# annegnx/PnP-Flow

Hardware: AMD Instinct MI355X
Metric: restored images/sec (higher is better)
Workload: dtype f32-equivalent (f16 hi+lo split operands, 3 x f16 MFMA per product, f32 accumulate); 1 GPU; CelebA-shaped 256x256 box-inpainting (half-size 40, sigma 0.05) pnp_flow B=32/GPU 100x5 (the configuration BASELINE.json's metric is quoted on; main.py:132-136 at 256^2); image=256x256x3, batch_per_gpu=32, global_batch=32, steps_pnp=100, num_samples=5, weights=synthetic seed 0 (no checkpoint offline), hipgraph=True, unet_batch=160, parallelism=dp1 (contiguous shards of the global batch, no data-path collective)

## Files before the change

pnpflow_amd/csrc/conv_pp.hip:

```cpp
#include "pp_common.h"

namespace pf {

constexpr int pp_a9(int MT) { return (pp_npix(MT) * 8 + 255) / 256; }

#ifdef PP_PROBE_BUILD
__device__ unsigned long long* g_pp_dbg = nullptr;
__device__ int g_pp_dbg_skip = 0;
#define PP_STAMP(k) do { if (stamp_buf != nullptr && blockIdx.x == 0 && t == 0 && stamp_n >= 0 && stamp_n < 64) stamp_buf[(team * 64 + stamp_n) * 8 + (k)] = __builtin_readcyclecounter(); } while (0)
#else
#define PP_STAMP(k) do { } while (0)
#endif

template <int MT, int N9, int N1, bool RES, int TEAMS = 2, int TERMS = 3>
__global__ __launch_bounds__(256 * TEAMS, 2) void conv_pp_kernel(const PPParams p) {
    constexpr int NCH = N9 + N1;
    constexpr int W9 = pp_w9(TERMS), W1 = pp_w1(TERMS), WSTEP = TERMS == 3 ? 2048 : 1024;
    static_assert(TERMS == 3 || TERMS == 1, "split terms");
    constexpr int PP_NPIX = pp_npix(MT), PP_PATCH_BYTES = pp_patch_bytes(MT), PP_A9 = pp_a9(MT), TH = 8 * MT;
    constexpr int LASTN = PP_NPIX * 8 - (PP_A9 - 1) * 256;
    constexpr int WBYTES = N9 * W9 + N1 * W1;
    static_assert(NCH >= 1 && NCH <= PP_MAXCH && N9 >= 1, "chunk structure");
    extern __shared__ __attribute__((aligned(16))) char smem[];
    const int tid = threadIdx.x;
    const int team = TEAMS == 2 ? __builtin_amdgcn_readfirstlane(tid >> 8) : 0;
    const int t = tid & 255, lane = t & 63, wm = __builtin_amdgcn_readfirstlane(t >> 6);
    const int l31 = lane & 31, hi = lane >> 5;
    const unsigned patch0 = (unsigned)WBYTES + (unsigned)team * PP_PATCH_BYTES;
    const pp_float_cptr scale_c = (pp_float_cptr)(uintptr_t)p.scale;
    auto wlds = [](int c) constexpr { return c < N9 ? c * W9 : N9 * W9 + (c - N9) * W1; };

#pragma unroll
    for (int c = 0; c < NCH; ++c) {
        const uint4* src = reinterpret_cast<const uint4*>(p.ch[c].wimg);
        uint4* dst = reinterpret_cast<uint4*>(smem + wlds(c));
        const int n16 = (c < N9 ? 9 : 1) * 256;
        if constexpr (TERMS == 3) {
            for (int i = tid; i < n16; i += 256 * TEAMS) dst[i] = src[i];
        } else {
            for (int i = tid; i < n16 / 2; i += 256 * TEAMS) dst[i] = src[(i >> 6) * 128 + (i & 63)];
        }
    }

    const int qi = t & 7, p0 = t >> 3;
    unsigned pk9[PP_A9];
#pragma unroll
    for (int i = 0; i < PP_A9; ++i) {
        const int pp = min(p0 + 32 * i, PP_NPIX - 1);
        const int py = pp / PP_PW, px = pp - py * PP_PW;
// ... 26 lines not shown

    const int G = gridDim.x;
    const int rg = (blockIdx.x & 7) * (G >> 3) + (blockIdx.x >> 3);
    const int T = p.B << (p.lx + p.ly);
    const int t_begin = (int)((long)rg * T / G), t_end = (int)((long)(rg + 1) * T / G);
    const int ntl = t_end - t_begin;
    const int niter = (ntl + TEAMS - 1) / TEAMS;
    const int rot = ntl > 0 ? (int)(((long)rg * p.rot) % ntl) : 0;
    auto tile_of = [&](int it) __attribute__((always_inline)) -> PPTile {
        const int idx = min(it * TEAMS + team, ntl - 1);
        const int wrapped = idx + rot >= ntl ? idx + rot - ntl : idx + rot;
        const int tl = t_begin + wrapped;
        PPTile r;
        const int tx = tl & ((1 << p.lx) - 1), ty = (tl >> p.lx) & ((1 << p.ly) - 1);
        r.b = tl >> (p.lx + p.ly); r.oy0 = ty * TH; r.ox0 = tx * 16;
        r.edge = (ty == 0 ? 1 : 0) | (ty == (1 << p.ly) - 1 ? 2 : 0) | (tx == 0 ? 4 : 0) | (tx == (1 << p.lx) - 1 ? 8 : 0);
        return r;
    };
    auto live_of = [&](int it) __attribute__((always_inline)) -> bool { return it >= 0 && (t_begin + it * TEAMS + team) < t_end; };

    struct Pre {
        float4 ra[PP_A9];
        float4 csc, csh;
        float ascale;
        unsigned inval;
    };
    Pre pre0, pre1;
    struct Res { float4 rv[MT][4]; float addv; };
    static_assert(MT == 1, "conv_pp_kernel: the residual / accumulator scheme below is the one of 8 x 16-pixel team tiles");
    constexpr int RD = 2;
    constexpr int NRES = NCH == 1 ? 2 : 1;
    Res res0, res1;

    auto issue_patch = [&](Pre& S, const PPTile& tl, auto C_) __attribute__((always_inline)) {
        constexpr int C = decltype(C_)::value;
        const long bpix = ((long)tl.b * p.H + tl.oy0) * p.W + tl.ox0;
        const int cstride = p.ch[C].cstride;
        S.ascale = p.scale != nullptr ? scale_c[8 * tl.b + p.ch[C].seg] : 1.0f;
        const unsigned cs4 = (unsigned)cstride * 4u, q16 = (unsigned)qi * 16u;
        if constexpr (C < N9) {
            const char* base = reinterpret_cast<const char*>(p.ch[C].src + (bpix - p.W - 1) * cstride + p.ch[C].coff);
            unsigned inval = 0;
#pragma unroll
            for (int i = 0; i < PP_A9; ++i) inval |= (((pk9[i] >> 20) & (unsigned)tl.edge) != 0u ? 1u : 0u) << i;
            S.inval = inval;
            const char* cb = reinterpret_cast<const char*>(p.coef + (size_t)tl.b * 2 * p.coef_stride + p.ch[C].gn_c0);
            S.csc = *reinterpret_cast<const float4*>(cb + q16); S.csh = *reinterpret_cast<const float4*>(cb + (unsigned)(p.coef_stride * 4) + q16);
#pragma unroll
            for (int i = 0; i < PP_A9; ++i) {
                const unsigned px = ((inval >> i) & 1u) ? (unsigned)pix_safe : (pk9[i] & 0xffffu);
                S.ra[i] = *reinterpret_cast<const float4*>(base + (__umul24(px, cs4) + q16));
            }
        } else {
            const char* base = reinterpret_cast<const char*>(p.ch[C].src + bpix * cstride + p.ch[C].coff);
            S.inval = 0;
#pragma unroll
            for (int i = 0; i < TH / 2; ++i) S.ra[i] = *reinterpret_cast<const float4*>(base + (__umul24((unsigned)(pixoff1 + 2 * i * p.W), cs4) + q16));
        }
    };

    auto split_store = [&](float4 v, unsigned addr) __attribute__((always_inline)) {
        if constexpr (TERMS == 3) {
            uint2 h, l;
            split4_pp(v, h.x, h.y, l.x, l.y);
            *reinterpret_cast<uint2*>(smem + addr) = h;
            *reinterpret_cast<uint2*>(smem + (addr ^ 64u)) = l;
        } else {
            uint2 h;
            asm("v_cvt_pk_f16_f32 %0, %2, %3\n\tv_cvt_pk_f16_f32 %1, %4, %5" : "=&v"(h.x), "=&v"(h.y) : "v"(v.x), "v"(v.y), "v"(v.z), "v"(v.w));
            *reinterpret_cast<uint2*>(smem + addr) = h;
        }
    };

    auto stage_and_request = [&](Pre& S, auto C_, const PPTile& t2, auto C2_) __attribute__((always_inline)) {
        constexpr int C = decltype(C_)::value, C2 = decltype(C2_)::value;
        constexpr int NT_ = C < N9 ? PP_A9 : TH / 2, NL_ = C2 < N9 ? PP_A9 : TH / 2;
        const long bpix = ((long)t2.b * p.H + t2.oy0) * p.W + t2.ox0;
        const int cstride = p.ch[C2].cstride;
        const unsigned cs4 = (unsigned)cstride * 4u, q16 = (unsigned)qi * 16u;
        const char* base = reinterpret_cast<const char*>(p.ch[C2].src + (bpix - (C2 < N9 ? p.W + 1 : 0)) * cstride + p.ch[C2].coff);
        unsigned inval2 = 0;
        if constexpr (C2 < N9) {
#pragma unroll
            for (int i = 0; i < PP_A9; ++i) inval2 |= (((pk9[i] >> 20) & (unsigned)t2.edge) != 0u ? 1u : 0u) << i;
        }
        const bool silu = C < N9 ? p.ch[C].xform == 2 : false;
#pragma unroll
        for (int i = 0; i < (NT_ > NL_ ? NT_ : NL_); ++i) {
            if (i < NT_) {
                float4 v = S.ra[i];
                if constexpr (C < N9) {
                    v.x = v.x * S.csc.x + S.csh.x; v.y = v.y * S.csc.y + S.csh.y; v.z = v.z * S.csc.z + S.csh.z; v.w = v.w * S.csc.w + S.csh.w;
                    if (silu) silu4_pp(v);
                    const float f = ((S.inval >> i) & 1u) ? 0.0f : S.ascale;
                    v.x *= f; v.y *= f; v.z *= f; v.w *= f;
                    if (i < PP_A9 - 1 || t < LASTN) split_store(v, ldsw9 + (unsigned)(i * 4096) + (((pk9[i] >> 16) & 7u) << 4));
                } else {
                    v.x *= S.ascale; v.y *= S.ascale; v.z *= S.ascale; v.w *= S.ascale;
                    split_store(v, ldsw1 + (unsigned)(2 * i * PP_PW * 128));
                }
            }
            if (i < NL_) {
                if constexpr (C2 < N9) {
                    const unsigned px = ((inval2 >> i) & 1u) ? (unsigned)pix_safe : (pk9[i] & 0xffffu);
                    S.ra[i] = *reinterpret_cast<const float4*>(base + (__umul24(px, cs4) + q16));
                } else {
                    S.ra[i] = *reinterpret_cast<const float4*>(base + (__umul24((unsigned)(pixoff1 + 2 * i * p.W), cs4) + q16));
                }
            }
        }
        S.inval = inval2;
        S.ascale = p.scale != nullptr ? scale_c[8 * t2.b + p.ch[C2].seg] : 1.0f;
        if constexpr (C2 < N9) {
            const char* cb = reinterpret_cast<const char*>(p.coef + (size_t)t2.b * 2 * p.coef_stride + p.ch[C2].gn_c0);
            S.csc = *reinterpret_cast<const float4*>(cb + q16); S.csh = *reinterpret_cast<const float4*>(cb + (unsigned)(p.coef_stride * 4) + q16);
        }
    };

    constexpr int NACC = 2;
    f32x16 acc[NACC][MT];
#pragma unroll
    for (int mt = 0; mt < MT; ++mt)
#pragma unroll
        for (int r = 0; r < 16; ++r) { for (int a = 0; a < NACC; ++a) acc[a][mt][r] = 0.f; }
    float run1[4] = {0.f, 0.f, 0.f, 0.f}, run2[4] = {0.f, 0.f, 0.f, 0.f};
    int run_b = -1, run_n = 0;

    auto mma_step = [&](unsigned wbase, int s, int ky, int kx, int j) __attribute__((always_inline)) {
        const int ai = (s & 1) % NACC;
        if constexpr (TERMS == 3) {
            const f16x8 bh = *reinterpret_cast<const f16x8*>(smem + wbase + (unsigned)((s * 2 + 0) * 1024));
            const f16x8 bl = *reinterpret_cast<const f16x8*>(smem + wbase + (unsigned)((s * 2 + 1) * 1024));
            f16x8 ah[MT], al[MT];
#pragma unroll
            for (int mt = 0; mt < MT; ++mt) {
                const unsigned off = (unsigned)((mt * 2 + ky) * PP_PW * 128);
                ah[mt] = *reinterpret_cast<const f16x8*>(smem + a_addr[kx][j][0] + off);
                al[mt] = *reinterpret_cast<const f16x8*>(smem + a_addr[kx][j][1] + off);
            }
#pragma unroll
            for (int mt = 0; mt < MT; ++mt) acc[ai][mt] = __builtin_amdgcn_mfma_f32_32x32x16_f16(al[mt], bh, acc[ai][mt], 0, 0, 0);
#pragma unroll
            for (int mt = 0; mt < MT; ++mt) acc[ai][mt] = __builtin_amdgcn_mfma_f32_32x32x16_f16(ah[mt], bl, acc[ai][mt], 0, 0, 0);
#pragma unroll
            for (int mt = 0; mt < MT; ++mt) acc[ai][mt] = __builtin_amdgcn_mfma_f32_32x32x16_f16(ah[mt], bh, acc[ai][mt], 0, 0, 0);
        } else {
            const f16x8 bh = *reinterpret_cast<const f16x8*>(smem + wbase + (unsigned)(s * WSTEP));
#pragma unroll
            for (int mt = 0; mt < MT; ++mt) {
                const f16x8 ah = *reinterpret_cast<const f16x8*>(smem + a_addr[kx][j][0] + (unsigned)((mt * 2 + ky) * PP_PW * 128));
                acc[ai][mt] = __builtin_amdgcn_mfma_f32_32x32x16_f16(ah, bh, acc[ai][mt], 0, 0, 0);
            }
        }
    };

    auto flush_stats = [&]() __attribute__((always_inline)) {
        if (p.stats_out == nullptr || run_b < 0) return;
#pragma unroll
        for (int j = 0; j < 4; ++j) {
            double a = (double)run1[j], q = (double)run2[j];
            a += __shfl_xor(a, 8); q += __shfl_xor(q, 8);
            a += __shfl_xor(a, 16); q += __shfl_xor(q, 16);
            a += __shfl_xor(a, 32); q += __shfl_xor(q, 32);
            if (lane < 8) {
                double* dst = p.stats_out + ((size_t)run_b * 32 + em * 4 + j) * 2;
                unsafeAtomicAdd(dst, a); unsafeAtomicAdd(dst + 1, q);
            }
            run1[j] = 0.f; run2[j] = 0.f;
        }
        run_n = 0;
    };

    auto epilogue = [&](const Res& R, const PPTile& tl, bool live) __attribute__((always_inline)) {
        if (!live) return;
        if (tl.b != run_b || run_n >= 32) { flush_stats(); run_b = tl.b; }
        ++run_n;
        const float inv_last = p.scale != nullptr ? scale_c[8 * tl.b + 4 + p.ch[NCH - 1].seg] : 1.0f;
        const float oscale = p.out_scale * (1.0f / 256.0f) * inv_last;
        float* obase = p.out + (((size_t)tl.b * p.H + tl.oy0 + wm * 2 * MT) * p.W + tl.ox0) * 32;
#pragma unroll
        for (int mt = 0; mt < MT; ++mt) {
            float e[16];
#pragma unroll
            for (int r = 0; r < 16; ++r) e[r] = (NACC == 2 ? acc[0][mt][r] + acc[NACC - 1][mt][r] : acc[0][mt][r]) * oscale + R.addv;
#pragma unroll
            for (int g = 0; g < 4; ++g) {
                oct_transpose(e[4 * g], e[4 * g + 1], e[4 * g + 2], e[4 * g + 3], bit3);
                float4 v = make_float4(e[4 * g], e[4 * g + 1], e[4 * g + 2], e[4 * g + 3]);
                if constexpr (RES) {
                    const float rsc = p.res_scale; const float4 r4 = R.rv[mt][g];
                    v.x = fmaf(r4.x, rsc, v.x); v.y = fmaf(r4.y, rsc, v.y); v.z = fmaf(r4.z, rsc, v.z); v.w = fmaf(r4.w, rsc, v.w);
                }
                char* dst = reinterpret_cast<char*>(obase) + (size_t)((mt * 2 + (g >> 1)) * p.W) * 128 + (g & 1) * 1024 + e_lane;
                nt_store4(dst, v);
                run1[0] += v.x; run1[1] += v.y; run1[2] += v.z; run1[3] += v.w;
                run2[0] += v.x * v.x; run2[1] += v.y * v.y; run2[2] += v.z * v.z; run2[3] += v.w * v.w;
            }
        }
    };

    auto issue_res = [&](Res& R, const PPTile& tl) __attribute__((always_inline)) {
        R.addv = p.addvec != nullptr ? p.addvec[(size_t)tl.b * p.addvec_bs + ch_of_col] : 0.f;
        if constexpr (RES) {
            const char* rbase = reinterpret_cast<const char*>(p.residual + (((size_t)tl.b * p.H + tl.oy0 + wm * 2 * MT) * p.W + tl.ox0) * 32);
#pragma unroll
            for (int mt = 0; mt < MT; ++mt)
#pragma unroll
                for (int g = 0; g < 4; ++g)
                    R.rv[mt][g] = nt_load4(rbase + (size_t)((mt * 2 + (g >> 1)) * p.W) * 128 + (g & 1) * 1024 + e_lane);
        }
    };

    auto mma_chunk = [&](const PPTile& tl, auto C_) __attribute__((always_inline)) {
        constexpr int C = decltype(C_)::value;
        if constexpr (C == 0) {
#pragma unroll
            for (int mt = 0; mt < MT; ++mt)
#pragma unroll
                for (int r = 0; r < 16; ++r) { for (int a = 0; a < NACC; ++a) acc[a][mt][r] = 0.f; }
        } else {
            if (p.scale != nullptr && p.ch[C - 1].seg != p.ch[C].seg) {
                const float ratio = scale_c[8 * tl.b + p.ch[C].seg] * scale_c[8 * tl.b + 4 + p.ch[C - 1].seg];
                if (ratio != 1.0f) {
#pragma unroll
                    for (int mt = 0; mt < MT; ++mt)
#pragma unroll
                        for (int r = 0; r < 16; ++r) { for (int a = 0; a < NACC; ++a) acc[a][mt][r] *= ratio; }
                }
            }
        }
        const unsigned wbase = (unsigned)wlds(C) + b_lane;
        __builtin_amdgcn_s_setprio(1);
        if constexpr (C < N9) {
#pragma unroll
            for (int tap = 0; tap < 9; ++tap)
#pragma unroll
                for (int j = 0; j < 2; ++j) mma_step(wbase, tap * 2 + j, tap / 3, tap % 3, j);
        } else {
#pragma unroll
            for (int j = 0; j < 2; ++j) mma_step(wbase, j, 1, 1, j);
        }
        __builtin_amdgcn_s_setprio(0);
    };

    int stamp_n = 0; (void)stamp_n;
#ifdef PP_PROBE_BUILD
    unsigned long long* const stamp_buf = g_pp_dbg;
    stamp_n = -g_pp_dbg_skip;
    if (stamp_buf != nullptr && (blockIdx.x & 31) == 0 && tid == 0) stamp_buf[2 * 64 * 8 + 2 * (blockIdx.x >> 5)] = __builtin_readcyclecounter();
#endif
    auto step = [&](int it, auto PAR_, auto C_, bool last_step) __attribute__((always_inline)) {
        constexpr int PAR = decltype(PAR_)::value, C = decltype(C_)::value;
        constexpr int SI = (NCH % 2 == 0) ? (C & 1) : ((PAR + C) & 1);
        Pre& S = SI == 0 ? pre0 : pre1;
        const PPTile tl = tile_of(it);
        PP_STAMP(0);
        PP_STAMP(1);
        if constexpr (C == 0) epilogue((NRES == 2 && (PAR ^ 1) == 1) ? res1 : res0, tile_of(it - 1), live_of(it - 1) && it > 0);
        PP_STAMP(2);
        constexpr int C2 = (C + 2) % NCH, DT = (C + 2) / NCH;
        stage_and_request(S, C_, tile_of(it + DT), ic<C2>{});
        PP_STAMP(3);
        constexpr int CR = (C + RD) % NCH, DTR = (C + RD) / NCH;
        if constexpr (CR == 0) issue_res((NRES == 2 && ((PAR + DTR - 1) & 1) == 1) ? res1 : res0, tile_of(it + DTR - 1));
        PP_STAMP(4);
        __syncthreads();
        PP_STAMP(5);
        mma_chunk(tl, C_);
        PP_STAMP(6);
        if (!(TEAMS == 2 && team == 1 && last_step)) __syncthreads();
        PP_STAMP(7);
        ++stamp_n;
    };
    auto tile_steps = [&](int it, auto PAR_) __attribute__((always_inline)) {
        const bool last_tile = it == niter - 1;
        if constexpr (NCH >= 1) step(it, PAR_, ic<0>{}, last_tile && NCH == 1);
        if constexpr (NCH >= 2) step(it, PAR_, ic<1>{}, last_tile && NCH == 2);
        if constexpr (NCH >= 3) step(it, PAR_, ic<2>{}, last_tile && NCH == 3);
        if constexpr (NCH >= 4) step(it, PAR_, ic<3>{}, last_tile && NCH == 4);
        if constexpr (NCH >= 5) step(it, PAR_, ic<4>{}, last_tile && NCH == 5);
        if constexpr (NCH >= 6) step(it, PAR_, ic<5>{}, last_tile && NCH == 6);
    };

    if (ntl <= 0) return;
    issue_patch(pre0, tile_of(0), ic<0>{});
    if constexpr (NCH == 1) { issue_patch(pre1, tile_of(1), ic<0>{}); if constexpr (RD == 2) issue_res(res0, tile_of(0)); }
    else issue_patch(pre1, tile_of(0), ic<1>{});
    __syncthreads();
    if (TEAMS == 2 && team == 1) __syncthreads();
    int it = 0;
    for (; it + 1 < niter; it += 2) {
        tile_steps(it, ic<0>{});
        tile_steps(it + 1, ic<1>{});
    }
    if (it < niter) tile_steps(it, ic<0>{});
    if (NRES == 2 && ((niter - 1) & 1)) epilogue(res1, tile_of(niter - 1), live_of(niter - 1));
    else epilogue(res0, tile_of(niter - 1), live_of(niter - 1));
    flush_stats();
#ifdef PP_PROBE_BUILD
    if (stamp_buf != nullptr && (blockIdx.x & 31) == 0 && tid == 0) stamp_buf[2 * 64 * 8 + 2 * (blockIdx.x >> 5) + 1] = __builtin_readcyclecounter();
#endif
}


template <int N9, int N1, bool RES, int TERMS>
static hipError_t launch_pp_t(const PPParams& p0, const ConvRoute& r, hipStream_t s) {
    constexpr int TEAMS = pp_teams(N9, N1, TERMS);
    static_assert(pp_structure(N9, N1, RES), "conv_route.h never routes this chunk structure");
    if (r.teams != TEAMS || r.grid_x <= 0) return hipErrorInvalidConfiguration;
    static unsigned long long attr_set = 0ull;
    auto kern = conv_pp_kernel<PP_MT, N9, N1, RES, TEAMS, TERMS>;
    { hipError_t e = set_max_dynamic_lds_once(reinterpret_cast<const void*>(kern), attr_set, ROUTE_LDS_MAX); if (e != hipSuccess) return e; }
    PPParams p = p0;
    p.lx = ilog2_exact(p.W / 16); p.ly = ilog2_exact(p.H / (8 * PP_MT));
    p.rot = 5;
    hipLaunchKernelGGL(kern, dim3(r.grid_x), dim3(256 * TEAMS), r.lds_bytes, s, p);
    return hipGetLastError();
}

hipError_t launch_conv_pp(const PPParams& p, const ConvRoute& r, hipStream_t s) {
    if (r.family != ConvFamily::PP || r.n9 != p.n9 || r.n1 != p.n1 || r.res != (p.residual != nullptr) || (r.terms != 3 && r.terms != 1)) return hipErrorInvalidValue;
#define PF_PP(n9_, n1_, res_) if (r.n9 == n9_ && r.n1 == n1_ && r.res == res_) return r.terms == 3 ? launch_pp_t<n9_, n1_, res_, 3>(p, r, s) : launch_pp_t<n9_, n1_, res_, 1>(p, r, s)
    PF_PP(1, 0, true); PF_PP(1, 0, false); PF_PP(2, 0, false); PF_PP(3, 0, false); PF_PP(1, 2, false); PF_PP(1, 3, false);
#undef PF_PP
    return hipErrorInvalidValue;
}

}
```

pnpflow_amd/csrc/engine.hip:

```cpp
#include <algorithm>
#include <cmath>
#include <cstdio>
#include <cstring>
#include <cstdlib>
#include <functional>
#include <map>
#include <memory>
#include <string>
#include <vector>

#include "../../include/pnpflow_hip.h"
#include "pf_common.h"
#include "weight_pack.h"
#include "rk45_control.h"
#include "adam_step.h"

using namespace pf;

namespace {

struct HostTensor { std::vector<int64_t> shape; std::vector<float> data; bool loaded = false; };

struct ResDesc {
    std::string prefix;
// ... 428 lines not shown
        const ConvSeg& sg = p.seg[i];
        const pf_engine::W16Src& src = e->w16_src.at(sg.w16);
        const wpack::Oihw w = oihw(e, src.name);
        for (int cc = 0; cc < sg.C / kc; ++cc) {
            PPChunk& k = q.ch[n++];
            k.src = sg.src; k.cstride = sg.cstride; k.coff = sg.coff + cc * kc; k.xform = sg.xform;
            k.gn_c0 = sg.gn_off + cc * kc; k.seg = i;
            const std::string& wn = src.name; const int lo = src.lo + cc * kc;
            const std::string sp_key = wn + (terms == 1 ? "#sph" : "#sp") + std::to_string(p.Cout) + "_" + std::to_string(lo);
            k.wimg = !sp ? weight_image(e, wn + "#pp" + std::to_string(lo), [&] { return wpack::chunk_pp(w, lo); })
                         : weight_image(e, r.nsplit == 2 ? sp_key + "_h0" : sp_key, [&] { return wpack::chunk_sp(w, lo, r.NT, terms, 0); });
            if (!k.wimg) return false;
            if (r.nsplit == 2) {
                q.wimg_h1[n - 1] = weight_image(e, sp_key + "_h1", [&] { return wpack::chunk_sp(w, lo, r.NT, terms, 128); });
                if (!q.wimg_h1[n - 1]) return false;
            }
            (sg.taps == 9 ? q.n9 : q.n1) += 1;
        }
    }
    q.B = p.B; q.H = p.H; q.W = p.W;
    q.out = p.out; q.addvec = p.addvec; q.addvec_bs = p.addvec_bs; q.residual = p.residual; q.res_scale = p.res_scale;
    q.stats_out = p.stats_out; q.out_scale = p.out_scale; q.coef = p.coef; q.coef_stride = p.coef_stride; q.scale = p.scale;
    return true;
}

static ConvFamily push_conv(Builder& bd, const ConvParams& p0, int stride = 1, int up = 0) {
    pf_engine* e = bd.e;
    ConvParams p = with_coef(bd, p0, bd.plan->ops);
    Op op{}; op.kind = OP_CONV;
    op.route = conv_route(routed_shape(e, p), stride, up, conv_terms(e), route_env());
    const ConvFamily f = op.route.family;
    bool built = true;
    if (op.route.refused) { built = false; e->err = std::string("conv launch refused: ") + op.route.refused; }
    else if (f == ConvFamily::PP || f == ConvFamily::SP) built = attach_pp(bd, p, op.route, op.ppp);
    else if (f == ConvFamily::DMA) built = attach_dma(bd, p, op.route, bd.plan->ops);
    if (!built) {
        if (bd.ok) { bd.ok = false; if (!op.route.refused) e->err = "conv launch: a weight image or operand buffer could not be allocated"; }
        return f;
    }
    op.cp = p; op.stride = stride; op.up = up; op.flops = conv_flops(p);
    bd.plan->gemm_flops += op.flops;
    bd.plan->ops.push_back(op);
    return f;
}


static Tensor res_block(Builder& bd, const ResDesc& r, const Tensor& in0, const Tensor* in1, float* temb_vec) {
    pf_engine* e = bd.e; const int B = bd.B, H = in0.H, Wd = in0.W;
    const int cin = in0.C + (in1 ? in1->C : 0);
    Tensor h1 = bd.make(r.cout, H, Wd, true);
    {
        ConvParams p = base_params(B, H, Wd, H, Wd, h1);
        packed_seg(e, p, in0, 2, 9, 0, r.prefix + "conv1.weight", 0, in0.C);
        if (in1) packed_seg(e, p, *in1, 2, 9, in0.C, r.prefix + "conv1.weight", in0.C, cin);
        p.gn_C = cin; p.gn_cpg = cin / 32;
        p.gamma = upload(e, r.prefix + "norm1.weight", W(e, r.prefix + "norm1.weight").data);
        p.beta = upload(e, r.prefix + "norm1.bias", W(e, r.prefix + "norm1.bias").data);
        p.addvec = temb_vec + e->temb_off.at(r.prefix); p.addvec_bs = e->temb_total;
        push_conv(bd, p);
    }
    Tensor out = bd.make(r.cout, H, Wd, true);
    {
        ConvParams p = base_params(B, H, Wd, H, Wd, out);
        packed_seg(e, p, h1, 2, 9, 0, r.prefix + "conv2.weight", 0, r.cout);
        p.gn_C = r.cout; p.gn_cpg = r.cout / 32;
        p.gamma = upload(e, r.prefix + "norm2.weight", W(e, r.prefix + "norm2.weight").data);
        p.beta = upload(e, r.prefix + "norm2.bias", W(e, r.prefix + "norm2.bias").data);
// ... 1505 lines not shown
```

pnpflow_amd/csrc/pf_common.h:

```cpp
#pragma once
#include <hip/hip_runtime.h>
#include <stdint.h>
#include <atomic>

#include "conv_route.h"
#include "deg_rules.h"

namespace pf {

inline hipError_t set_max_dynamic_lds_once(const void* kernel, unsigned long long& done, int bytes = 160 * 1024) {
    int dev = 0;
    hipError_t e = hipGetDevice(&dev);
    if (e != hipSuccess) return e;
    if (dev >= 0 && dev < 64 && ((done >> dev) & 1ull)) return hipSuccess;
    e = hipFuncSetAttribute(kernel, hipFuncAttributeMaxDynamicSharedMemorySize, bytes);
    if (e == hipSuccess && dev >= 0 && dev < 64) done |= 1ull << dev;
    return e;
}

inline int device_cu_count() {
    static std::atomic<int> cache[64] = {};
    int dev = 0;
    if (hipGetDevice(&dev) != hipSuccess) return 0;
    if (dev >= 0 && dev < 64) { const int c = cache[dev].load(std::memory_order_relaxed); if (c > 0) return c; }
// ... 90 lines not shown
    const float* bias;
    int B, H, W, Cimg, C;
    const double* stats; const float* gamma; const float* beta; int gn_cpg; float gn_eps;
    double* stats_out;
    const void* w16;
};

struct AttnParams { const float* qkv; float* out; int B, T, C; float scale; const float* bias; const float* residual; float* stats_part; int kv_packed; };
hipError_t launch_partial_stats(const float* part, double* stats, int B, int nparts, int C, hipStream_t s);
bool attn_fused_supported(int T, int C);
hipError_t launch_attn_fused(const AttnParams& p, hipStream_t s);

struct TembParams {
    const float* t;
    const float* w0; const float* b0;
    const float* w1; const float* b1;
    const float* wp;
    const float* bp;
    float* out;
    int B, ch, total_out;
};

struct GnCoefParams {
    const double* st[3];
    int C[3], xform[3], gn_off[3];
    int nseg, gn_C, gn_cpg, HW;
    float eps;
    const float* gamma; const float* beta;
    float* coef; int coef_stride;
    float* scale;
    unsigned int* flags;
    int id;
    float* mu_out; float* rs_out;
};
hipError_t launch_gn_coef(const GnCoefParams& p, int B, hipStream_t s);

struct PrepParams {
    const float* src[3]; void* dst[3];
    int C[3], cstride[3], coff[3], xform[3], gn_off[3];
    int nseg, B, Hs, Ws, terms;
    const float* coef; int coef_stride;
    const float* scale;
};
hipError_t launch_prep_split(const PrepParams& p, hipStream_t s);
hipError_t launch_conv_dma(const ConvParams& p, const ConvRoute& r, hipStream_t s);
size_t conv_dma_a16_bytes(int B, int C, int Hs, int Ws, int terms);

struct PPChunk {
    const float* src;
    const void* wimg;
    int cstride, coff;
    int xform;
    int gn_c0;
    int seg;
    int pad_;
};
struct PPParams {
    PPChunk ch[PP_MAXCH];
    int n9, n1;
    int cout;
    int B, H, W, lx, ly;
    int rot;
    float* out; const float* addvec; int addvec_bs; const float* residual; float res_scale; double* stats_out; float out_scale;
    const float* coef; int coef_stride; const float* scale;
    const void* wimg_h1[PP_MAXCH];
};
hipError_t launch_conv_pp(const PPParams& p, const ConvRoute& r, hipStream_t s);
hipError_t launch_conv_sp(const PPParams& p, const ConvRoute& r, hipStream_t s);
hipError_t launch_conv(const ConvParams& p, const ConvRoute& r, hipStream_t s);
hipError_t launch_conv16(const ConvParams& p, const ConvRoute& r, hipStream_t s);
size_t conv_flops(const ConvParams& p);
hipError_t launch_begin_conv(const EdgeConvParams& p, hipStream_t s);
hipError_t launch_end_conv(const EdgeConvParams& p, hipStream_t s);
hipError_t launch_temb(const TembParams& p, hipStream_t s);
hipError_t launch_softmax_rows(float* data, int64_t rows, int cols, hipStream_t s);

hipError_t launch_gn_fwd_coeffs(const double* st0, int C0, const double* st1, int C1, int cpg, int HW, float eps, float* mu, float* rs, int B,
                                hipStream_t s);
hipError_t launch_gn_bwd_pre(float* g, const float* x, const float* mu, const float* rs, const float* gamma, const float* beta, double* bsum,
                             int B, int HW, int C, int coff, int Ct, int silu, hipStream_t s);
hipError_t launch_gn_bwd_coeffs(const double* bsum, int Ct, int cpg, int HW, float* m1, float* m2, int B, hipStream_t s);
hipError_t launch_gn_bwd_post(const float* dy, const float* x, const float* mu, const float* rs, const float* m1, const float* m2,
                              const float* add, float* out, int B, int HW, int C, int coff, int Ct, int accumulate, hipStream_t s, float add_scale = 1.0f);
hipError_t launch_transpose(const float* in, float* out, int B, int R, int Cc, hipStream_t s);
hipError_t launch_softmax_bwd(const float* A, float* dA, int64_t rows, int cols, float scale, hipStream_t s);
hipError_t launch_sumpool2(const float* in, float* out, int B, int H, int W, int C, int accumulate, hipStream_t s);

hipError_t launch_deg_H(const DegView& d, const float* x, float* y, int B, int C, int H, int W, float* scratch, hipStream_t s);
hipError_t launch_deg_Hadj(const DegView& d, const float* y, float* x, int B, int C, int H, int W, float* scratch, hipStream_t s);
hipError_t launch_grad_step(const DegView& d, const float* x, const float* y, const float* coef, float* z,
                            int B, int C, int H, int W, float* scratch, int laplace, hipStream_t s);
hipError_t launch_psf_sr(const DegView& d, const float* in, float* out, int B, int C, int H, int W, int sign, int mode, const float* aux, const float* coef,
                         hipStream_t s);
hipError_t launch_psf2d(const DegView& d, const float* in, float* out, int B, int C, int H, int W, int sign, int mode, const float* aux, const float* coef,
                        hipStream_t s);
hipError_t launch_psf_power_spectrum(const DegView& d, int H, int W, float* pw2, hipStream_t s);
hipError_t launch_interpolate(const float* z, const float* t, const float* noise, uint64_t seed, uint64_t stream_id,
                              float* zt, int B, int n, hipStream_t s);
hipError_t launch_interp_iter(const float* z, const float* t, const float* noise, const unsigned long long* rng ,
                              const int* iter, int num_samples, int sample, float* zt, int B, int n, hipStream_t s);
// ... 109 lines not shown
```

pnpflow_amd/csrc/pp_common.h:

```cpp
#pragma once
#include "pf_common.h"

namespace pf {

typedef float f32x16 __attribute__((ext_vector_type(16)));
typedef _Float16 f16x8 __attribute__((ext_vector_type(8)));
typedef _Float16 f16x4 __attribute__((ext_vector_type(4)));

typedef const __attribute__((address_space(4))) float* pp_float_cptr;

__device__ __forceinline__ float silu_pp(float x) { return x * __builtin_amdgcn_rcpf(1.0f + __expf(-x)); }

__device__ __forceinline__ void silu4_pp(float4& v) {
    float t0, t1, t2, t3;
    asm("v_mul_f32 %4, 0xbfb8aa3b, %0\n\tv_mul_f32 %5, 0xbfb8aa3b, %1\n\tv_mul_f32 %6, 0xbfb8aa3b, %2\n\tv_mul_f32 %7, 0xbfb8aa3b, %3\n\t"
        "v_exp_f32 %4, %4\n\tv_exp_f32 %5, %5\n\tv_exp_f32 %6, %6\n\tv_exp_f32 %7, %7\n\t"
        "v_add_f32 %4, 1.0, %4\n\tv_add_f32 %5, 1.0, %5\n\tv_add_f32 %6, 1.0, %6\n\tv_add_f32 %7, 1.0, %7\n\t"
        "v_rcp_f32 %4, %4\n\tv_rcp_f32 %5, %5\n\tv_rcp_f32 %6, %6\n\tv_rcp_f32 %7, %7\n\t"
        "v_mul_f32 %0, %0, %4\n\tv_mul_f32 %1, %1, %5\n\tv_mul_f32 %2, %2, %6\n\tv_mul_f32 %3, %3, %7"
        : "+v"(v.x), "+v"(v.y), "+v"(v.z), "+v"(v.w), "=&v"(t0), "=&v"(t1), "=&v"(t2), "=&v"(t3));
}

__device__ __forceinline__ void split4_pp(const float4& v, unsigned& h01, unsigned& h23, unsigned& l01, unsigned& l23) {
    asm("v_cvt_pk_f16_f32 %0, %4, %5\n\tv_cvt_pk_f16_f32 %1, %6, %7\n\t"
        "v_fma_mixlo_f16 %2, %0, -1.0, %4 op_sel_hi:[1,0,0]\n\t"
        "v_fma_mixlo_f16 %3, %1, -1.0, %6 op_sel_hi:[1,0,0]\n\t"
        "v_fma_mixhi_f16 %2, %0, -1.0, %5 op_sel:[1,0,0] op_sel_hi:[1,0,0]\n\t"
        "v_fma_mixhi_f16 %3, %1, -1.0, %7 op_sel:[1,0,0] op_sel_hi:[1,0,0]"
        : "=&v"(h01), "=&v"(h23), "=&v"(l01), "=&v"(l23) : "v"(v.x), "v"(v.y), "v"(v.z), "v"(v.w));
}

typedef float pp_f4v __attribute__((ext_vector_type(4)));
__device__ __forceinline__ void nt_store4(void* dst, const float4& v) { pp_f4v t_ = {v.x, v.y, v.z, v.w}; __builtin_nontemporal_store(t_, reinterpret_cast<pp_f4v*>(dst)); }
__device__ __forceinline__ float4 nt_load4(const void* src) { const pp_f4v t_ = __builtin_nontemporal_load(reinterpret_cast<const pp_f4v*>(src)); return make_float4(t_.x, t_.y, t_.z, t_.w); }

template <int CTRL>
__device__ __forceinline__ float dpp_quad(float v) {
    return __builtin_bit_cast(float, __builtin_amdgcn_update_dpp(0, __builtin_bit_cast(int, v), CTRL, 0xf, 0xf, true));
}

__device__ __forceinline__ void oct_transpose(float& a0, float& a1, float& a2, float& a3, bool bit3) {
    constexpr int ROR8 = 0x128;
    float b0 = a0, b1 = a1, b2 = a2, b3 = a3;
    asm("s_nop 1\n\tv_permlane16_swap_b32 %0, %1\n\tv_permlane16_swap_b32 %2, %3\n\ts_nop 1" : "+v"(b0), "+v"(b2), "+v"(b1), "+v"(b3));
    const float d0 = dpp_quad<ROR8>(b0), d1 = dpp_quad<ROR8>(b1), d2 = dpp_quad<ROR8>(b2), d3 = dpp_quad<ROR8>(b3);
    a0 = bit3 ? d1 : b0; a1 = bit3 ? b1 : d0; a2 = bit3 ? d3 : b2; a3 = bit3 ? b3 : d2;
}

struct PPTile { int b, oy0, ox0, edge; };
template <int K> struct ic { static constexpr int value = K; };

}
```

pnpflow_amd/csrc/unet_misc.hip:

```cpp
#include "pf_common.h"

namespace pf {

__device__ __forceinline__ float silu_acc(float x) { return x / (1.0f + expf(-x)); }

template <int C>
__global__ __launch_bounds__(256) void begin_conv_kernel(const EdgeConvParams p) {
    __shared__ float s_t[256][C + 1];
    __shared__ float s_part[8][C][2];
    const int tid = threadIdx.x;
    const float* __restrict__ wgt = p.w;
    const float* __restrict__ bias = p.bias;
    const int HW = p.H * p.W;
    const int pix0 = blockIdx.x * 256;
    const int pix = pix0 + tid;
    const int b = blockIdx.y;
    const bool valid = pix < HW;
    float acc[C];
#pragma unroll
    for (int c = 0; c < C; ++c) acc[c] = valid ? bias[c] : 0.f;
    if (valid) {
        const int y = pix / p.W, x = pix % p.W;
        for (int ci = 0; ci < p.Cimg; ++ci) {
            const float* img = p.in + ((size_t)b * p.Cimg + ci) * HW;
// ... 432 lines not shown
    for (int i = lane; i < cols; i += 64) r[i] *= inv;
}

hipError_t launch_softmax_rows(float* data, int64_t rows, int cols, hipStream_t s) {
    hipLaunchKernelGGL(softmax_rows_kernel, dim3((unsigned)((rows + 3) / 4)), dim3(256), 0, s, data, rows, cols);
    return hipGetLastError();
}

__global__ __launch_bounds__(256) void gn_coef_kernel(const GnCoefParams p) {
    __shared__ double s_st[2 * 1024];
    __shared__ double s_red[16];
    __shared__ int s_bad;
    const int b = blockIdx.x, tid = threadIdx.x;
    if (tid == 0) s_bad = 0;
    bool bad = false;
    for (int c = tid; c < p.gn_C; c += 256) {
        double a = 0.0, q = 0.0;
        for (int si = 0; si < p.nseg; ++si)
            if (p.xform[si] != 0 && c >= p.gn_off[si] && c < p.gn_off[si] + p.C[si]) {
                const double* st = p.st[si] + ((size_t)b * p.C[si] + (c - p.gn_off[si])) * 2;
                a = st[0]; q = st[1];
            }
        bad |= !(isfinite(a) && isfinite(q));
        s_st[2 * c] = a; s_st[2 * c + 1] = q;
    }
    double raw_ss[3] = {0.0, 0.0, 0.0};
    for (int si = 0; si < p.nseg; ++si)
        if (p.xform[si] == 0 && p.st[si] != nullptr)
            for (int c = tid; c < p.C[si]; c += 256) {
                const double q = p.st[si][((size_t)b * p.C[si] + c) * 2 + 1];
                bad |= !isfinite(q);
                raw_ss[si] += q;
            }
    __syncthreads();
    double gn_ms = 0.0;
    const double inv_n = 1.0 / ((double)p.gn_cpg * (double)p.HW);
    for (int c = tid; c < p.gn_C; c += 256) {
        const int g0 = (c / p.gn_cpg) * p.gn_cpg;
        double sm = 0.0, ss = 0.0;
        for (int j = g0; j < g0 + p.gn_cpg; ++j) { sm += s_st[2 * j]; ss += s_st[2 * j + 1]; }
        const double mean = sm * inv_n;
        double var = ss * inv_n - mean * mean;
        var = var > 0.0 ? var : 0.0;
        const float rstd = (float)(1.0 / sqrt(var + (double)p.eps));
        const float ga = p.gamma[c], be = p.beta[c];
        const float sc = ga * rstd;
        p.coef[((size_t)b * 2 + 0) * p.coef_stride + c] = sc;
        p.coef[((size_t)b * 2 + 1) * p.coef_stride + c] = be - (float)mean * sc;
        if (p.mu_out != nullptr) { p.mu_out[(size_t)b * p.gn_C + c] = (float)mean; p.rs_out[(size_t)b * p.gn_C + c] = rstd; }
        gn_ms += (double)ga * ga + (double)be * be;
    }
    if (bad) atomicOr(&s_bad, 1);
    if (p.scale != nullptr) {
#pragma unroll
        for (int o = 32; o > 0; o >>= 1) {
            gn_ms += __shfl_xor(gn_ms, o);
#pragma unroll
            for (int k = 0; k < 3; ++k) raw_ss[k] += __shfl_xor(raw_ss[k], o);
        }
        if ((tid & 63) == 0) { s_red[(tid >> 6) * 4] = gn_ms; for (int k = 0; k < 3; ++k) s_red[(tid >> 6) * 4 + 1 + k] = raw_ss[k]; }
    }
    __syncthreads();
    if (tid == 0) {
        if (s_bad && p.flags != nullptr) { atomicOr(p.flags, 1u); atomicCAS(p.flags + 1, 0u, (unsigned)(p.id + 1)); }
        if (p.scale != nullptr) {
            auto pow2_for = [](double ms) {
                float s = 1.0f;
                const float rms = (float)sqrt(ms);
                if (isfinite(rms) && rms > 0.f && (rms < 0.25f || rms > 64.f)) {
                    int e; frexpf(rms, &e);
                    e = e < -40 ? -40 : (e > 40 ? 40 : e);
                    s = ldexpf(1.0f, -e);
                }
                return s;
            };
            const double gs = s_red[0] + s_red[4] + s_red[8] + s_red[12];
            const float s_gn = p.gn_C > 0 ? pow2_for(gs / (double)p.gn_C) : 1.0f;
            for (int si = 0; si < 3; ++si) {
                float sv = 1.0f;
                if (si < p.nseg) {
                    if (p.xform[si] != 0) sv = s_gn;
                    else if (p.st[si] != nullptr)
                        sv = pow2_for((s_red[1 + si] + s_red[5 + si] + s_red[9 + si] + s_red[13 + si]) / ((double)p.C[si] * (double)p.HW));
                }
                p.scale[8 * b + si] = sv; p.scale[8 * b + 4 + si] = 1.0f / sv;
            }
        }
    }
}

hipError_t launch_gn_coef(const GnCoefParams& p, int B, hipStream_t s) {
    if (p.gn_C > 1024 || (p.gn_C > 0 && (p.coef == nullptr || p.gn_cpg <= 0))) return hipErrorInvalidValue;
    hipLaunchKernelGGL(gn_coef_kernel, dim3(B), dim3(256), 0, s, p);
    return hipGetLastError();
}

}
```

Measured before the change: 3.477 images/s.

## Add lean conv_pp path folding power-of-two scale into GroupNorm coefficients

Adds a LEAN instantiation of the pointer-patch conv kernel for the two-chunk 3x3 non-residual case. The GroupNorm coefficient kernel now pre-multiplies scale and shift by the power-of-two activation scale. The lean kernel folds that scale into the SiLU exponent constant, so the per-element scale multiply goes away. It also adds a branch-free interior-tile path that skips edge masking, plus cheaper 32-bit shift-based address math. This trims VALU work in the staging loop, at the cost of extra template instantiations, code size and register pressure, and it needs B*H*W to fit in 32 bits.

```diff
diff --git a/pnpflow_amd/csrc/conv_pp.hip b/pnpflow_amd/csrc/conv_pp.hip
--- a/pnpflow_amd/csrc/conv_pp.hip
+++ b/pnpflow_amd/csrc/conv_pp.hip
@@ -12,9 +12,19 @@
 #define PP_STAMP(k) do { } while (0)
 #endif
 
-template <int MT, int N9, int N1, bool RES, int TEAMS = 2, int TERMS = 3>
+#ifndef PP_LEAN_PARTS
+constexpr int pp_lean_parts(int N9, int N1, bool RES, int TERMS) { return N9 == 2 && N1 == 0 && !RES && TERMS == 3 ? 7 : 0; }
+#else
+constexpr int pp_lean_parts(int N9, int N1, bool RES, int TERMS) {
+    return (N9 == 3 && TERMS == 3 ? 0 : (N9 == 1 && N1 == 0 && RES && TERMS == 3 ? 5 : 7)) & PP_LEAN_PARTS;
+}
+#endif
+template <int MT, int N9, int N1, bool RES, int TEAMS = 2, int TERMS = 3, bool LEAN = true>
 __global__ __launch_bounds__(256 * TEAMS, 2) void conv_pp_kernel(const PPParams p) {
     constexpr int NCH = N9 + N1;
+    constexpr int LPARTS = LEAN ? pp_lean_parts(N9, N1, RES, TERMS) : 0;
+    constexpr bool L_FOLD = (LPARTS & 1) != 0, L_INT = (LPARTS & 2) != 0, L_ADDR = (LPARTS & 4) != 0;
+    static_assert(!LEAN || L_FOLD, "a LEAN instantiation reads pre-scaled coefficients: part 1 is what makes it one");
     constexpr int W9 = pp_w9(TERMS), W1 = pp_w1(TERMS), WSTEP = TERMS == 3 ? 2048 : 1024;
     static_assert(TERMS == 3 || TERMS == 1, "split terms");
     constexpr int PP_NPIX = pp_npix(MT), PP_PATCH_BYTES = pp_patch_bytes(MT), PP_A9 = pp_a9(MT), TH = 8 * MT;
@@ -107,19 +117,47 @@
     constexpr int NRES = NCH == 1 ? 2 : 1;
     Res res0, res1;
 
+    auto pre_scalar = [&](int b, auto C_) __attribute__((always_inline)) -> float {
+        constexpr int C = decltype(C_)::value;
+        if constexpr (L_FOLD && C < N9) {
+            constexpr unsigned NLOG2E = 0xbfb8aa3bu;
+            return __uint_as_float(p.scale != nullptr ? __float_as_uint(scale_c[8 * b + 4 + p.ch[C].seg]) + (NLOG2E - 0x3f800000u) : NLOG2E);
+        } else {
+            return p.scale != nullptr ? scale_c[8 * b + p.ch[C].seg] : 1.0f;
+        }
+    };
+    auto tile_pix = [&](const PPTile& tl) __attribute__((always_inline)) -> unsigned {
+        return ((((unsigned)tl.b << (p.ly + 3)) + (unsigned)tl.oy0) << (p.lx + 4)) + (unsigned)tl.ox0;
+    };
+    auto patch_base = [&](const PPTile& tl, auto C_) __attribute__((always_inline)) -> const char* {
+        constexpr int C = decltype(C_)::value;
+        const unsigned cs4 = (unsigned)p.ch[C].cstride * 4u;
+        const long off = (long)((unsigned long)tile_pix(tl) * cs4) - (C < N9 ? (long)((unsigned)(p.W + 1) * cs4) : 0l);
+        return reinterpret_cast<const char*>(p.ch[C].src + p.ch[C].coff) + off;
+    };
+    auto coef_base = [&](int b, auto C_) __attribute__((always_inline)) -> const char* {
+        constexpr int C = decltype(C_)::value;
+        if constexpr (L_ADDR) return reinterpret_cast<const char*>(p.coef + p.ch[C].gn_c0) + (unsigned long)(unsigned)b * ((unsigned)p.coef_stride * 8u);
+        else return reinterpret_cast<const char*>(p.coef + (size_t)b * 2 * p.coef_stride + p.ch[C].gn_c0);
+    };
+    auto out_pix = [&](const PPTile& tl) __attribute__((always_inline)) -> size_t { return (size_t)(tile_pix(tl) + ((unsigned)(wm * 2 * MT) << (p.lx + 4))); };
+
     auto issue_patch = [&](Pre& S, const PPTile& tl, auto C_) __attribute__((always_inline)) {
         constexpr int C = decltype(C_)::value;
         const long bpix = ((long)tl.b * p.H + tl.oy0) * p.W + tl.ox0;
         const int cstride = p.ch[C].cstride;
-        S.ascale = p.scale != nullptr ? scale_c[8 * tl.b + p.ch[C].seg] : 1.0f;
+        if constexpr (LEAN) S.ascale = pre_scalar(tl.b, C_);
+        else S.ascale = p.scale != nullptr ? scale_c[8 * tl.b + p.ch[C].seg] : 1.0f;
         const unsigned cs4 = (unsigned)cstride * 4u, q16 = (unsigned)qi * 16u;
         if constexpr (C < N9) {
             const char* base = reinterpret_cast<const char*>(p.ch[C].src + (bpix - p.W - 1) * cstride + p.ch[C].coff);
+            if constexpr (L_ADDR) base = patch_base(tl, C_);
             unsigned inval = 0;
 #pragma unroll
             for (int i = 0; i < PP_A9; ++i) inval |= (((pk9[i] >> 20) & (unsigned)tl.edge) != 0u ? 1u : 0u) << i;
             S.inval = inval;
             const char* cb = reinterpret_cast<const char*>(p.coef + (size_t)tl.b * 2 * p.coef_stride + p.ch[C].gn_c0);
+            if constexpr (L_ADDR) cb = coef_base(tl.b, C_);
             S.csc = *reinterpret_cast<const float4*>(cb + q16); S.csh = *reinterpret_cast<const float4*>(cb + (unsigned)(p.coef_stride * 4) + q16);
 #pragma unroll
             for (int i = 0; i < PP_A9; ++i) {
@@ -128,6 +166,7 @@
             }
         } else {
             const char* base = reinterpret_cast<const char*>(p.ch[C].src + bpix * cstride + p.ch[C].coff);
+            if constexpr (L_ADDR) base = patch_base(tl, C_);
             S.inval = 0;
 #pragma unroll
             for (int i = 0; i < TH / 2; ++i) S.ra[i] = *reinterpret_cast<const float4*>(base + (__umul24((unsigned)(pixoff1 + 2 * i * p.W), cs4) + q16));
@@ -192,6 +231,71 @@
         }
     };
 
+    auto stage_and_request_lean = [&](Pre& S, auto C_, int edge_st, const PPTile& t2, auto C2_) __attribute__((always_inline)) {
+        constexpr int C = decltype(C_)::value, C2 = decltype(C2_)::value;
+        constexpr int NT_ = C < N9 ? PP_A9 : TH / 2, NL_ = C2 < N9 ? PP_A9 : TH / 2;
+        const long bpix = ((long)t2.b * p.H + t2.oy0) * p.W + t2.ox0;
+        const int cstride = p.ch[C2].cstride;
+        const unsigned cs4 = (unsigned)cstride * 4u, q16 = (unsigned)qi * 16u;
+        const char* base = L_ADDR ? patch_base(t2, C2_) : reinterpret_cast<const char*>(p.ch[C2].src + (bpix - (C2 < N9 ? p.W + 1 : 0)) * cstride + p.ch[C2].coff);
+        const bool silu = C < N9 ? p.ch[C].xform == 2 : false;
+        auto body = [&](auto INT_) __attribute__((always_inline)) {
+            constexpr bool INT = decltype(INT_)::value != 0;
+            unsigned inval2 = 0;
+            if constexpr (C2 < N9 && !INT) {
+#pragma unroll
+                for (int i = 0; i < PP_A9; ++i) inval2 |= (((pk9[i] >> 20) & (unsigned)t2.edge) != 0u ? 1u : 0u) << i;
+            }
+#pragma unroll
+            for (int i = 0; i < (NT_ > NL_ ? NT_ : NL_); ++i) {
+                if (i < NT_) {
+                    float4 v = S.ra[i];
+                    if constexpr (C < N9) {
+                        v.x = v.x * S.csc.x + S.csh.x; v.y = v.y * S.csc.y + S.csh.y; v.z = v.z * S.csc.z + S.csh.z; v.w = v.w * S.csc.w + S.csh.w;
+                        if constexpr (L_FOLD) {
+                            if (silu) silu4_pp(v, S.ascale);
+                            if constexpr (!INT) {
+                                const float f = ((S.inval >> i) & 1u) ? 0.0f : 1.0f;
+                                v.x *= f; v.y *= f; v.z *= f; v.w *= f;
+                            }
+                        } else {
+                            if (silu) silu4_pp(v);
+                            if constexpr (!INT) {
+                                const float f = ((S.inval >> i) & 1u) ? 0.0f : S.ascale;
+                                v.x *= f; v.y *= f; v.z *= f; v.w *= f;
+                            } else {
+                                v.x *= S.ascale; v.y *= S.ascale; v.z *= S.ascale; v.w *= S.ascale;
+                            }
+                        }
+                        if (i < PP_A9 - 1 || t < LASTN) split_store(v, ldsw9 + (unsigned)(i * 4096) + (((pk9[i] >> 16) & 7u) << 4));
+                    } else {
+                        v.x *= S.ascale; v.y *= S.ascale; v.z *= S.ascale; v.w *= S.ascale;
+                        split_store(v, ldsw1 + (unsigned)(2 * i * PP_PW * 128));
+                    }
+                }
+                if (i < NL_) {
+                    if constexpr (C2 < N9) {
+                        const unsigned px = INT ? (pk9[i] & 0xffffu) : (((inval2 >> i) & 1u) ? (unsigned)pix_safe : (pk9[i] & 0xffffu));
+                        S.ra[i] = *reinterpret_cast<const float4*>(base + (__umul24(px, cs4) + q16));
+                    } else {
+                        S.ra[i] = *reinterpret_cast<const float4*>(base + (__umul24((unsigned)(pixoff1 + 2 * i * p.W), cs4) + q16));
+                    }
+                }
+            }
+            S.inval = inval2;
+        };
+        if constexpr (L_INT && (C < N9 || C2 < N9)) {
+            if ((C < N9 ? edge_st == 0 : true) && (C2 < N9 ? t2.edge == 0 : true)) body(ic<1>{}); else body(ic<0>{});
+        } else {
+            body(ic<0>{});
+        }
+        S.ascale = pre_scalar(t2.b, C2_);
+        if constexpr (C2 < N9) {
+            const char* cb = coef_base(t2.b, C2_);
+            S.csc = *reinterpret_cast<const float4*>(cb + q16); S.csh = *reinterpret_cast<const float4*>(cb + (unsigned)(p.coef_stride * 4) + q16);
+        }
+    };
+
     constexpr int NACC = 2;
     f32x16 acc[NACC][MT];
 #pragma unroll
@@ -253,6 +357,7 @@
         const float inv_last = p.scale != nullptr ? scale_c[8 * tl.b + 4 + p.ch[NCH - 1].seg] : 1.0f;
         const float oscale = p.out_scale * (1.0f / 256.0f) * inv_last;
         float* obase = p.out + (((size_t)tl.b * p.H + tl.oy0 + wm * 2 * MT) * p.W + tl.ox0) * 32;
+        if constexpr (L_ADDR) obase = p.out + out_pix(tl) * 32;
 #pragma unroll
         for (int mt = 0; mt < MT; ++mt) {
             float e[16];
@@ -278,6 +383,7 @@
         R.addv = p.addvec != nullptr ? p.addvec[(size_t)tl.b * p.addvec_bs + ch_of_col] : 0.f;
         if constexpr (RES) {
             const char* rbase = reinterpret_cast<const char*>(p.residual + (((size_t)tl.b * p.H + tl.oy0 + wm * 2 * MT) * p.W + tl.ox0) * 32);
+            if constexpr (L_ADDR) rbase = reinterpret_cast<const char*>(p.residual + out_pix(tl) * 32);
 #pragma unroll
             for (int mt = 0; mt < MT; ++mt)
 #pragma unroll
@@ -334,7 +440,8 @@
         if constexpr (C == 0) epilogue((NRES == 2 && (PAR ^ 1) == 1) ? res1 : res0, tile_of(it - 1), live_of(it - 1) && it > 0);
         PP_STAMP(2);
         constexpr int C2 = (C + 2) % NCH, DT = (C + 2) / NCH;
-        stage_and_request(S, C_, tile_of(it + DT), ic<C2>{});
+        if constexpr (LEAN) stage_and_request_lean(S, C_, tl.edge, tile_of(it + DT), ic<C2>{});
+        else stage_and_request(S, C_, tile_of(it + DT), ic<C2>{});
         PP_STAMP(3);
         constexpr int CR = (C + RD) % NCH, DTR = (C + RD) / NCH;
         if constexpr (CR == 0) issue_res((NRES == 2 && ((PAR + DTR - 1) & 1) == 1) ? res1 : res0, tile_of(it + DTR - 1));
@@ -378,13 +485,13 @@
 }
 
 
-template <int N9, int N1, bool RES, int TERMS>
+template <int N9, int N1, bool RES, int TERMS, bool LEAN>
 static hipError_t launch_pp_t(const PPParams& p0, const ConvRoute& r, hipStream_t s) {
     constexpr int TEAMS = pp_teams(N9, N1, TERMS);
     static_assert(pp_structure(N9, N1, RES), "conv_route.h never routes this chunk structure");
     if (r.teams != TEAMS || r.grid_x <= 0) return hipErrorInvalidConfiguration;
     static unsigned long long attr_set = 0ull;
-    auto kern = conv_pp_kernel<PP_MT, N9, N1, RES, TEAMS, TERMS>;
+    auto kern = conv_pp_kernel<PP_MT, N9, N1, RES, TEAMS, TERMS, LEAN>;
     { hipError_t e = set_max_dynamic_lds_once(reinterpret_cast<const void*>(kern), attr_set, ROUTE_LDS_MAX); if (e != hipSuccess) return e; }
     PPParams p = p0;
     p.lx = ilog2_exact(p.W / 16); p.ly = ilog2_exact(p.H / (8 * PP_MT));
@@ -393,9 +500,18 @@
     return hipGetLastError();
 }
 
+template <int N9, int N1, bool RES, int TERMS>
+static hipError_t launch_pp_lean(const PPParams& p, const ConvRoute& r, hipStream_t s) {
+    if constexpr (pp_lean_parts(N9, N1, RES, TERMS) != 0) { if (p.lean) return launch_pp_t<N9, N1, RES, TERMS, true>(p, r, s); }
+    return launch_pp_t<N9, N1, RES, TERMS, false>(p, r, s);
+}
+
+bool conv_pp_lean(const ConvRoute& r) { return r.family == ConvFamily::PP && pp_lean_parts(r.n9, r.n1, r.res, r.terms) != 0; }
+
 hipError_t launch_conv_pp(const PPParams& p, const ConvRoute& r, hipStream_t s) {
     if (r.family != ConvFamily::PP || r.n9 != p.n9 || r.n1 != p.n1 || r.res != (p.residual != nullptr) || (r.terms != 3 && r.terms != 1)) return hipErrorInvalidValue;
-#define PF_PP(n9_, n1_, res_) if (r.n9 == n9_ && r.n1 == n1_ && r.res == res_) return r.terms == 3 ? launch_pp_t<n9_, n1_, res_, 3>(p, r, s) : launch_pp_t<n9_, n1_, res_, 1>(p, r, s)
+    if (p.lean && (!conv_pp_lean(r) || (unsigned long long)p.B * p.H * p.W > 0xffffffffull)) return hipErrorInvalidValue;
+#define PF_PP(n9_, n1_, res_) if (r.n9 == n9_ && r.n1 == n1_ && r.res == res_) return r.terms == 3 ? launch_pp_lean<n9_, n1_, res_, 3>(p, r, s) : launch_pp_lean<n9_, n1_, res_, 1>(p, r, s)
     PF_PP(1, 0, true); PF_PP(1, 0, false); PF_PP(2, 0, false); PF_PP(3, 0, false); PF_PP(1, 2, false); PF_PP(1, 3, false);
 #undef PF_PP
     return hipErrorInvalidValue;
diff --git a/pnpflow_amd/csrc/engine.hip b/pnpflow_amd/csrc/engine.hip
--- a/pnpflow_amd/csrc/engine.hip
+++ b/pnpflow_amd/csrc/engine.hip
@@ -484,7 +484,14 @@
     const ConvFamily f = op.route.family;
     bool built = true;
     if (op.route.refused) { built = false; e->err = std::string("conv launch refused: ") + op.route.refused; }
-    else if (f == ConvFamily::PP || f == ConvFamily::SP) built = attach_pp(bd, p, op.route, op.ppp);
+    else if (f == ConvFamily::PP || f == ConvFamily::SP) {
+        built = attach_pp(bd, p, op.route, op.ppp);
+        static const bool lean_env = !(getenv("PNPFLOW_HIP_PP_LEAN") && atoi(getenv("PNPFLOW_HIP_PP_LEAN")) == 0);
+        if (built && f == ConvFamily::PP && lean_env && conv_pp_lean(op.route) && p.coef != nullptr && !bd.plan->ops.empty() && bd.plan->ops.back().kind == OP_GN_COEF) {
+            bd.plan->ops.back().gp.prescale = 1;
+            op.ppp.lean = 1;
+        }
+    }
     else if (f == ConvFamily::DMA) built = attach_dma(bd, p, op.route, bd.plan->ops);
     if (!built) {
         if (bd.ok) { bd.ok = false; if (!op.route.refused) e->err = "conv launch: a weight image or operand buffer could not be allocated"; }
diff --git a/pnpflow_amd/csrc/pf_common.h b/pnpflow_amd/csrc/pf_common.h
--- a/pnpflow_amd/csrc/pf_common.h
+++ b/pnpflow_amd/csrc/pf_common.h
@@ -146,6 +146,7 @@
     unsigned int* flags;
     int id;
     float* mu_out; float* rs_out;
+    int prescale;
 };
 hipError_t launch_gn_coef(const GnCoefParams& p, int B, hipStream_t s);
 
@@ -178,8 +179,10 @@
     float* out; const float* addvec; int addvec_bs; const float* residual; float res_scale; double* stats_out; float out_scale;
     const float* coef; int coef_stride; const float* scale;
     const void* wimg_h1[PP_MAXCH];
+    int lean;
 };
 hipError_t launch_conv_pp(const PPParams& p, const ConvRoute& r, hipStream_t s);
+bool conv_pp_lean(const ConvRoute& r);
 hipError_t launch_conv_sp(const PPParams& p, const ConvRoute& r, hipStream_t s);
 hipError_t launch_conv(const ConvParams& p, const ConvRoute& r, hipStream_t s);
 hipError_t launch_conv16(const ConvParams& p, const ConvRoute& r, hipStream_t s);
diff --git a/pnpflow_amd/csrc/pp_common.h b/pnpflow_amd/csrc/pp_common.h
--- a/pnpflow_amd/csrc/pp_common.h
+++ b/pnpflow_amd/csrc/pp_common.h
@@ -19,6 +19,16 @@
         "v_rcp_f32 %4, %4\n\tv_rcp_f32 %5, %5\n\tv_rcp_f32 %6, %6\n\tv_rcp_f32 %7, %7\n\t"
         "v_mul_f32 %0, %0, %4\n\tv_mul_f32 %1, %1, %5\n\tv_mul_f32 %2, %2, %6\n\tv_mul_f32 %3, %3, %7"
         : "+v"(v.x), "+v"(v.y), "+v"(v.z), "+v"(v.w), "=&v"(t0), "=&v"(t1), "=&v"(t2), "=&v"(t3));
+}
+
+__device__ __forceinline__ void silu4_pp(float4& v, float nlog2e) {
+    float t0, t1, t2, t3;
+    asm("v_mul_f32 %4, %8, %0\n\tv_mul_f32 %5, %8, %1\n\tv_mul_f32 %6, %8, %2\n\tv_mul_f32 %7, %8, %3\n\t"
+        "v_exp_f32 %4, %4\n\tv_exp_f32 %5, %5\n\tv_exp_f32 %6, %6\n\tv_exp_f32 %7, %7\n\t"
+        "v_add_f32 %4, 1.0, %4\n\tv_add_f32 %5, 1.0, %5\n\tv_add_f32 %6, 1.0, %6\n\tv_add_f32 %7, 1.0, %7\n\t"
+        "v_rcp_f32 %4, %4\n\tv_rcp_f32 %5, %5\n\tv_rcp_f32 %6, %6\n\tv_rcp_f32 %7, %7\n\t"
+        "v_mul_f32 %0, %0, %4\n\tv_mul_f32 %1, %1, %5\n\tv_mul_f32 %2, %2, %6\n\tv_mul_f32 %3, %3, %7"
+        : "+v"(v.x), "+v"(v.y), "+v"(v.z), "+v"(v.w), "=&v"(t0), "=&v"(t1), "=&v"(t2), "=&v"(t3) : "s"(nlog2e));
 }
 
 __device__ __forceinline__ void split4_pp(const float4& v, unsigned& h01, unsigned& h23, unsigned& l01, unsigned& l23) {
diff --git a/pnpflow_amd/csrc/unet_misc.hip b/pnpflow_amd/csrc/unet_misc.hip
--- a/pnpflow_amd/csrc/unet_misc.hip
+++ b/pnpflow_amd/csrc/unet_misc.hip
@@ -488,8 +488,30 @@
                 bad |= !isfinite(q);
                 raw_ss[si] += q;
             }
-    __syncthreads();
     double gn_ms = 0.0;
+    if (p.scale != nullptr) {
+        for (int c = tid; c < p.gn_C; c += 256) { const float ga = p.gamma[c], be = p.beta[c]; gn_ms += (double)ga * ga + (double)be * be; }
+#pragma unroll
+        for (int o = 32; o > 0; o >>= 1) {
+            gn_ms += __shfl_xor(gn_ms, o);
+#pragma unroll
+            for (int k = 0; k < 3; ++k) raw_ss[k] += __shfl_xor(raw_ss[k], o);
+        }
+        if ((tid & 63) == 0) { s_red[(tid >> 6) * 4] = gn_ms; for (int k = 0; k < 3; ++k) s_red[(tid >> 6) * 4 + 1 + k] = raw_ss[k]; }
+    }
+    __syncthreads();
+    auto pow2_for = [](double ms) {
+        float s = 1.0f;
+        const float rms = (float)sqrt(ms);
+        if (isfinite(rms) && rms > 0.f && (rms < 0.25f || rms > 64.f)) {
+            int e; frexpf(rms, &e);
+            e = e < -40 ? -40 : (e > 40 ? 40 : e);
+            s = ldexpf(1.0f, -e);
+        }
+        return s;
+    };
+    const float s_gn = p.scale != nullptr && p.gn_C > 0 ? pow2_for((s_red[0] + s_red[4] + s_red[8] + s_red[12]) / (double)p.gn_C) : 1.0f;
+    const float pre = p.prescale ? s_gn : 1.0f;
     const double inv_n = 1.0 / ((double)p.gn_cpg * (double)p.HW);
     for (int c = tid; c < p.gn_C; c += 256) {
         const int g0 = (c / p.gn_cpg) * p.gn_cpg;
@@ -501,37 +523,16 @@
         const float rstd = (float)(1.0 / sqrt(var + (double)p.eps));
         const float ga = p.gamma[c], be = p.beta[c];
         const float sc = ga * rstd;
-        p.coef[((size_t)b * 2 + 0) * p.coef_stride + c] = sc;
-        p.coef[((size_t)b * 2 + 1) * p.coef_stride + c] = be - (float)mean * sc;
+        const float sh = be - (float)mean * sc;
+        p.coef[((size_t)b * 2 + 0) * p.coef_stride + c] = sc * pre;
+        p.coef[((size_t)b * 2 + 1) * p.coef_stride + c] = sh * pre;
         if (p.mu_out != nullptr) { p.mu_out[(size_t)b * p.gn_C + c] = (float)mean; p.rs_out[(size_t)b * p.gn_C + c] = rstd; }
-        gn_ms += (double)ga * ga + (double)be * be;
     }
     if (bad) atomicOr(&s_bad, 1);
-    if (p.scale != nullptr) {
-#pragma unroll
-        for (int o = 32; o > 0; o >>= 1) {
-            gn_ms += __shfl_xor(gn_ms, o);
-#pragma unroll
-            for (int k = 0; k < 3; ++k) raw_ss[k] += __shfl_xor(raw_ss[k], o);
-        }
-        if ((tid & 63) == 0) { s_red[(tid >> 6) * 4] = gn_ms; for (int k = 0; k < 3; ++k) s_red[(tid >> 6) * 4 + 1 + k] = raw_ss[k]; }
-    }
     __syncthreads();
     if (tid == 0) {
         if (s_bad && p.flags != nullptr) { atomicOr(p.flags, 1u); atomicCAS(p.flags + 1, 0u, (unsigned)(p.id + 1)); }
         if (p.scale != nullptr) {
-            auto pow2_for = [](double ms) {
-                float s = 1.0f;
-                const float rms = (float)sqrt(ms);
-                if (isfinite(rms) && rms > 0.f && (rms < 0.25f || rms > 64.f)) {
-                    int e; frexpf(rms, &e);
-                    e = e < -40 ? -40 : (e > 40 ? 40 : e);
-                    s = ldexpf(1.0f, -e);
-                }
-                return s;
-            };
-            const double gs = s_red[0] + s_red[4] + s_red[8] + s_red[12];
-            const float s_gn = p.gn_C > 0 ? pow2_for(gs / (double)p.gn_C) : 1.0f;
             for (int si = 0; si < 3; ++si) {
                 float sv = 1.0f;
                 if (si < p.nseg) {
```

Result: no change. 3.479 images/s (median of 3 runs) (+0.1%).
